# samuelkriegerbonini-dev/AstroBurst

Measured on AMD Instinct MI355X. Metric: MPix/s sigma-clipped stack+stretch, 64x4096x4096 f32, higher is better.
Workload: dtype f32

## Files before the change

### astroburst_amd/csrc/affine.hip

```cpp
#include "ab_common.hpp"

#include <algorithm>
#include <condition_variable>
#include <mutex>
#include <thread>
#include <array>
#include <atomic>
#include <chrono>
#include <cmath>
#include <thread>

int ab_phase_correlate_device(ab_ctx *ctx, const float *ref, int64_t ref_rows, int64_t ref_cols, int64_t ref_ld, const float *tgt,
                              int64_t tgt_rows, int64_t tgt_cols, int64_t tgt_ld, double *dx, double *dy, double *confidence);

namespace {

constexpr size_t kMaxStars = 120;
constexpr double kTriangleTolerance = 0.02;
constexpr size_t kMinMatchesAffine = 6, kMinMatchesRigid = 4;
constexpr size_t kRansacIterations = 2000;
constexpr double kRansacInlierPx = 3.0, kDetectionSigma = 3.5, kMinTriangleSide = 15.0;
constexpr uint32_t kMinVotes = 1;
constexpr double kMinInlierRatio = 0.20, kMaxResidualPx = 5.0, kMaxOffsetFraction = 0.40, kMaxRotationDeg = 30.0;
constexpr double kMinScale = 0.70, kMaxScale = 1.40;
// ... 373 lines not shown
    __syncthreads();
    if (ok) {
        unsigned int base = block_base;
        for (int w = 0; w < wv; ++w) base += wave_cnt[w];
        out[base + (unsigned int)__builtin_popcountll(m & ((1ull << lane) - 1ull))] = tri;
        if (bin_hist) atomicAdd(&lhist[tri.bin], 1u);
    }
    if (bin_hist) {
        __syncthreads();
        for (int b = threadIdx.x; b < kTriBins; b += kTriBlock)
            if (lhist[b]) atomicAdd(&bin_hist[b], lhist[b]);
    }
}

constexpr int kScanThreads = 256, kScanPer = kTriBins / kScanThreads;
__device__ __forceinline__ void tri_bin_scan_body(unsigned int *__restrict__ hist, unsigned int *__restrict__ off ,
                                                            unsigned int *__restrict__ cursor) {
    __shared__ unsigned int wave_tot[kScanThreads / 64];
    const int t = threadIdx.x, lane = t & 63, wv = t >> 6;
    unsigned int h[kScanPer], s = 0;
#pragma unroll
    for (int j = 0; j < kScanPer; j += 4) {
        const uint4 q = *reinterpret_cast<const uint4 *>(hist + kScanPer * t + j);
        h[j] = q.x, h[j + 1] = q.y, h[j + 2] = q.z, h[j + 3] = q.w;
        s += q.x + q.y + q.z + q.w;
    }
    unsigned int inc = s;
#pragma unroll
    for (int o = 1; o < 64; o <<= 1) {
        const unsigned int u = __shfl_up(inc, o, 64);
        if (lane >= o) inc += u;
    }
    if (lane == 63) wave_tot[wv] = inc;
    __syncthreads();
    unsigned int base = 0;
    for (int i = 0; i < wv; ++i) base += wave_tot[i];
    unsigned int e = base + inc - s;
#pragma unroll
    for (int j = 0; j < kScanPer; ++j) {
        off[kScanPer * t + j] = e;
        cursor[kScanPer * t + j] = e;
        hist[kScanPer * t + j] = 0;
        e += h[j];
    }
    if (t == kScanThreads - 1) off[kTriBins] = e;
}

__device__ __forceinline__ void tri_scatter_body(const DTri *__restrict__ in, const unsigned int *__restrict__ n_p, unsigned int *cursor,
                                                           DTri *__restrict__ sorted) {
    __shared__ unsigned int cnt[kTriBins];
    const unsigned int n = *n_p, i = blockIdx.x * kTriBlock + threadIdx.x;
    if (blockIdx.x * kTriBlock >= n) return;
    for (int b = threadIdx.x; b < kTriBins; b += kTriBlock) cnt[b] = 0;
    __syncthreads();
    DTri t = {0.0, 0.0, 0u, 0u};
    unsigned int rank = 0;
    if (i < n) {
// ... 165 lines not shown
    __syncthreads();
    unsigned int *mine = votes_out + (size_t)(blockIdx.x % (unsigned int)copies) * (kVoteDim * kVoteDim);
    for (int row = wv; row < kVoteDim; row += kVoteWaves) {
        const unsigned int v = votes[row * kVoteLdsStride + lane];
        if (v) atomicAdd(&mine[row * kVoteDim + lane], v);
    }
}

constexpr int kTriGroupMax = 8;
struct TriGroup {
    int n;
    int limit[kTriGroupMax];
    DTri *raw[kTriGroupMax], *sorted[kTriGroupMax];
    unsigned int *count[kTriGroupMax], *bin_hist[kTriGroupMax], *bin_off[kTriGroupMax], *cursor[kTriGroupMax], *votes[kTriGroupMax];
};
__global__ __launch_bounds__(kTriBlock) void tri_build_kernel(const StarXY stars, int limit, DTri *__restrict__ out, unsigned int *count,
                                                         unsigned int *__restrict__ bin_hist, unsigned int *__restrict__ votes_to_clear, int vote_words) { AB_LATENCY_KERNEL_PRIO();
    tri_build_body(stars.xy, limit, out, count, bin_hist, votes_to_clear, vote_words);
}
__global__ __launch_bounds__(kTriBlock) void tri_build_many_kernel(const TriGroup g, const StarXY *__restrict__ stars, int vote_words) { AB_LATENCY_KERNEL_PRIO();
    const int f = blockIdx.y;
    tri_build_body(stars[f].xy, g.limit[f], g.raw[f], g.count[f], g.bin_hist[f], g.votes[f], vote_words);
}
__global__ __launch_bounds__(kScanThreads) void tri_bin_scan_kernel(unsigned int *__restrict__ hist, unsigned int *__restrict__ off, unsigned int *__restrict__ cursor) { AB_LATENCY_KERNEL_PRIO();
    tri_bin_scan_body(hist, off, cursor);
}
__global__ __launch_bounds__(kScanThreads) void tri_bin_scan_many_kernel(const TriGroup g) { AB_LATENCY_KERNEL_PRIO();
    const int f = blockIdx.y;
    tri_bin_scan_body(g.bin_hist[f], g.bin_off[f], g.cursor[f]);
}
__global__ __launch_bounds__(kTriBlock) void tri_scatter_kernel(const DTri *__restrict__ in, const unsigned int *__restrict__ n_p, unsigned int *cursor,
                                                           DTri *__restrict__ sorted) { AB_LATENCY_KERNEL_PRIO();
    tri_scatter_body(in, n_p, cursor, sorted);
}
__global__ __launch_bounds__(kTriBlock) void tri_scatter_many_kernel(const TriGroup g) { AB_LATENCY_KERNEL_PRIO();
    const int f = blockIdx.y;
    tri_scatter_body(g.raw[f], g.count[f], g.cursor[f], g.sorted[f]);
}
__global__ __launch_bounds__(64) void tri_vote_kernel(const DTri *__restrict__ rt_sorted, const unsigned int *__restrict__ nr_p, const DTri *__restrict__ tt_sorted,
                                                      const unsigned int *__restrict__ bin_off, unsigned int *__restrict__ votes_out, int copies,
                                                      const RefGroup *__restrict__ groups, unsigned int *__restrict__ tgt_count_to_clear) { AB_LATENCY_KERNEL_PRIO();
    tri_vote_body(rt_sorted, nr_p, tt_sorted, bin_off, votes_out, copies, groups, tgt_count_to_clear);
}
__global__ __launch_bounds__(64) void tri_vote_many_kernel(const TriGroup g, const DTri *__restrict__ rt_sorted, const unsigned int *__restrict__ nr_p, int copies,
                                                           const RefGroup *__restrict__ groups) { AB_LATENCY_KERNEL_PRIO();
    const int f = blockIdx.y;
    tri_vote_body(rt_sorted, nr_p, g.sorted[f], g.bin_off[f], g.votes[f], copies, groups, g.count[f]);
}
__global__ __launch_bounds__(kVoteWaves * 64) void tri_vote_wide_kernel(const DTri *__restrict__ rt_sorted, const unsigned int *__restrict__ nr_p, const DTri *__restrict__ tt_sorted,
                                                                        const unsigned int *__restrict__ bin_off, unsigned int *__restrict__ votes_out, int copies,
                                                                        const RefGroup *__restrict__ groups, unsigned int *__restrict__ tgt_count_to_clear, unsigned int slices) { AB_LATENCY_KERNEL_PRIO();
    tri_vote_wide_body(rt_sorted, nr_p, tt_sorted, bin_off, votes_out, copies, groups, tgt_count_to_clear, slices);
}
__global__ __launch_bounds__(kVoteWaves * 64) void tri_vote_wide_many_kernel(const TriGroup g, const DTri *__restrict__ rt_sorted, const unsigned int *__restrict__ nr_p, int copies,
                                                                             const RefGroup *__restrict__ groups, unsigned int slices) { AB_LATENCY_KERNEL_PRIO();
    const int f = blockIdx.y;
    tri_vote_wide_body(rt_sorted, nr_p, g.sorted[f], g.bin_off[f], g.votes[f], copies, groups, g.count[f], slices);
}
unsigned int vote_wide_slices() {
    static const unsigned int v = [] {
        const char *e = ab_dev_env("AB_VOTE_SLICES");
        const int x = e ? atoi(e) : 8;
        return (unsigned int)(x < 1 ? 1 : (x > 8 ? 8 : x));
    }();
    return v;
}
bool vote_wide() {
    static const bool on = [] {
        const char *e = ab_dev_env("AB_VOTE_WAVES");
        return !(e && atoi(e) == 1);
    }();
    return on;
}

__global__ __launch_bounds__(256) void votes_reduce_many_kernel(const TriGroup g, int copies, uint32_t *__restrict__ out) { AB_LATENCY_KERNEL_PRIO();
    const int f = blockIdx.y, i = blockIdx.x * 256 + threadIdx.x;
    if (i >= kVoteDim * kVoteDim) return;
    uint32_t s = 0;
    for (int c = 0; c < copies; ++c) s += g.votes[f][(size_t)c * kVoteDim * kVoteDim + i];
    out[(size_t)f * kVoteDim * kVoteDim + i] = s;
}

struct MatchWs {
    DTri *ref_tris, *ref_sorted, *tgt_tris, *tgt_sorted;
    unsigned int *counts;
    unsigned int *bin_hist, *bin_off, *cursor;
    unsigned int *votes;
    RefGroup *groups;
};

int match_ws(ab_ctx *ctx, MatchWs *w) {
    const size_t tri_bytes = (size_t)kMaxTris * sizeof(DTri), vote_bytes = (size_t)kVoteCopiesMax * kVoteDim * kVoteDim * sizeof(unsigned int);
    const size_t bin_words = 64 + 3 * (size_t)kTriBins + 64;
    const size_t group_bytes = (size_t)((kMaxTris + 63) / 64) * sizeof(RefGroup);
    const size_t total = 4 * tri_bytes + bin_words * sizeof(unsigned int) + vote_bytes + group_bytes;
// ... 110 lines not shown
    int max_limit = 0;
    for (int f = 0; f < G; ++f) {
        const int limit = (int)std::min<size_t>(stars[f].size(), kTriLimit);
        w.g.limit[f] = limit;
        max_limit = std::max(max_limit, limit);
        for (int i = 0; i < limit; ++i) {
            hs[f].xy[2 * i] = stars[f][i][0];
            hs[f].xy[2 * i + 1] = stars[f][i][1];
        }
    }
    for (int f = 0; f < G; ++f) votes[f].assign((size_t)kVoteDim * kVoteDim, 0u);
    if (max_limit < 3) return AB_OK;
    AB_HIP(ctx, hipMemcpyAsync(w.stars, hs, stars_bytes, hipMemcpyHostToDevice, ctx->stream));
    const int total = max_limit * max_limit * max_limit, blocks = std::max((total + kTriBlock - 1) / kTriBlock, (vote_words + kTriBlock - 1) / kTriBlock);
    hipLaunchKernelGGL(tri_build_many_kernel, dim3(blocks, G), dim3(kTriBlock), 0, ctx->stream, w.g, (const StarXY *)w.stars, vote_words);
    hipLaunchKernelGGL(tri_bin_scan_many_kernel, dim3(1, G), dim3(kScanThreads), 0, ctx->stream, w.g);
    hipLaunchKernelGGL(tri_scatter_many_kernel, dim3((kMaxTris + kTriBlock - 1) / kTriBlock, G), dim3(kTriBlock), 0, ctx->stream, w.g);
    if (vote_wide())
        hipLaunchKernelGGL(tri_vote_wide_many_kernel, dim3((kVoteItemsMax + kVoteWaves - 1) / kVoteWaves, G), dim3(kVoteWaves * 64), 0, ctx->stream, w.g,
                           (const DTri *)ref_ws.ref_sorted, (const unsigned int *)ref_ws.counts, copies, (const RefGroup *)ref_ws.groups, vote_wide_slices());
    else
        hipLaunchKernelGGL(tri_vote_many_kernel, dim3(kVoteBlocks, G), dim3(64), 0, ctx->stream, w.g, (const DTri *)ref_ws.ref_sorted, (const unsigned int *)ref_ws.counts,
                           copies, (const RefGroup *)ref_ws.groups);
    uint32_t *hv = (uint32_t *)((char *)pin + stars_bytes);
    hipLaunchKernelGGL(votes_reduce_many_kernel, dim3((kVoteDim * kVoteDim + 255) / 256, G), dim3(256), 0, ctx->stream, w.g, copies, hv);
    AB_HIP(ctx, hipGetLastError());
    AB_HIP(ctx, hipStreamSynchronize(ctx->stream));
    for (int f = 0; f < G; ++f) votes[f].assign(hv + (size_t)f * per_frame_words, hv + (size_t)(f + 1) * per_frame_words);
    return AB_OK;
}

int frame_stars(ab_ctx *ctx, const float *img, int64_t rows, int64_t cols, std::vector<Pt> *out, const ab_pixel_xf *xf = nullptr,
                const double *bg = nullptr, const ab_frame_cand *cand = nullptr ) {
    std::vector<ab_detected_star> stars;
    double m, s;
    if (xf && bg) {
        const double b2[1][2] = {{bg[0], bg[1]}};
        AB_TRY(ab_detect_stars_group_device(ctx, &img, 1, rows, cols, kDetectionSigma, xf, b2, kMaxStars, &stars, cand));
    } else {
        AB_TRY(ab_detect_stars_device(ctx, img, rows, cols, cols, kDetectionSigma, &stars, &m, &s, xf ? *xf : ab_pixel_xf(), kMaxStars,
// ... 447 lines not shown
```

### astroburst_amd/csrc/detect.hip

```cpp
#include "ab_common.hpp"
#include "block_select.hpp"
#include "tile_bucket.hpp"
#include "tile_stream.hpp"

#include <algorithm>
#include <cfloat>
#include <cmath>
#include <chrono>
#include <condition_variable>
#include <thread>

namespace {

constexpr double kMadToSigma = 1.4826;

struct FrameDev {
    ab_pixel_xf xf;
    double bg_median, bg_sigma, threshold;
    unsigned int finite;
    unsigned int pad;
};

constexpr int kCandCap = 2048;
struct TileCand {
// ... 1356 lines not shown
    unsigned int *mask[kGroupMax], *counters[kGroupMax];
    CompStat *st[kGroupMax];
    CompRec *rec[kGroupMax];
    unsigned int ncomp[kGroupMax];
    unsigned int comp_cap;
    int chained;
    int *blist[kGroupMax];
    unsigned int *lcnt[kGroupMax];
    size_t plist_stride, blist_stride;
    int tiled;
    int mask_pitch;
    int recs;
    size_t rec_stride;
    unsigned int *sel[kGroupMax];
    unsigned int *selout[kGroupMax];
    const uint2 *cand_ent[kGroupMax];
    const unsigned int *cand_cnt[kGroupMax];
    const float *cand_cut[kGroupMax];
    int tile_h, tile_w;
};

static inline bool selection_cut_too_close(const std::vector<ab_detected_star> &stars, size_t max_keep, unsigned int selected, unsigned int candidates,
                                           unsigned int cut_key) {
    if (candidates <= selected || cut_key == 0 || stars.empty() || stars.size() < max_keep) return false;
    unsigned long long bits;
    const double fl = stars.back().flux;
    memcpy(&bits, &fl, sizeof bits);
    const unsigned long long key = (bits >> 32) + 1ull;
    return key < (unsigned long long)cut_key + 2ull;
}

constexpr unsigned int kSelKeep = 480, kSelCap = 544;
__device__ __forceinline__ unsigned int sel_key(const CompStat &c) {
    const bool ok = c.npix >= 3 && c.npix <= 5000 && c.first_interior != 0x7fffffff && c.flux > 0.0;
    return ok ? (unsigned int)((unsigned long long)__double_as_longlong(c.flux) >> 32) + 1u : 0u;
}
constexpr int kSelThreads = 256, kSelSub = 2048;
__device__ __forceinline__ unsigned int sel_digit(unsigned int k) {
    constexpr int kBase = (1023 - 64) << 20;
    const int d = ((int)k - kBase) >> 16;
    return (unsigned int)(d < 0 ? 0 : (d > 2047 ? 2047 : d));
}
__device__ __forceinline__ void sel_find_digit(const unsigned int *hist, int nb, unsigned int want, int tid, unsigned int *digit, unsigned int *above) {
    unsigned int run = 0, found = 0, ab = 0;
    bool done = false;
    for (int base = nb - 64; base >= 0 && !done; base -= 64) {
        const unsigned int c = hist[base + 63 - tid];
        unsigned int incl = c;
#pragma unroll
        for (int off = 1; off < 64; off <<= 1) {
            const unsigned int o = __shfl_up(incl, off, 64);
            if (tid >= off) incl += o;
        }
        const unsigned long long hit = __ballot(run + incl >= want);
        if (hit) {
            const int l = __builtin_ctzll(hit);
            ab = run + __shfl(incl, l, 64) - __shfl(c, l, 64);
            found = (unsigned int)(base + 63 - l);
            done = true;
        } else {
            run += __shfl(incl, 63, 64);
        }
    }
    *digit = found;
    *above = ab;
}
__global__ __launch_bounds__(kSelThreads) void comp_select_many_kernel(const DetGroup g) { AB_LATENCY_KERNEL_PRIO();
    const int f = blockIdx.x, tid = threadIdx.x;
    unsigned int n = g.ncomp[f];
    if (g.chained && !g.recs) {
        n = g.counters[f][0];
        if (tid == 0) g.selout[f][2] = n;
        if (n > g.comp_cap) n = 0;
    }
    const CompStat *__restrict__ st = g.st[f];
    unsigned int *__restrict__ sel = g.sel[f];
    __shared__ unsigned int hist[2048];
    __shared__ unsigned int sub_key[kSelSub], sub_idx[kSelSub];
    __shared__ unsigned int s_ncand, s_d0, s_above, s_count, s_nsub, s_prefix, s_want, s_ge, s_take;
    __shared__ unsigned int seg_n[kRecRegions], seg_t0[kRecRegions + 1];
    const int nseg = g.recs ? kRecRegions : 1;
    const unsigned int seg_stride = g.recs ? (unsigned int)g.rec_stride : 0u;
    for (unsigned int b = tid; b < 2048; b += kSelThreads) hist[b] = 0;
    if (tid == 0) s_ncand = s_d0 = s_above = s_count = s_nsub = s_prefix = s_want = s_ge = s_take = 0;
    if (g.recs) {
        const unsigned int flagw = g.counters[f][3];
        const bool overflow = (flagw & 1u) != 0;
        if (tid == 0 && g.chained) g.selout[f][4] = flagw >> 1;
        if (tid < kRecRegions) {
            const unsigned int cnt = g.lcnt[f][(2 * kRegions + tid) * kRegionPitch];
            seg_n[tid] = overflow ? 0u : (cnt < seg_stride ? cnt : seg_stride);
        }
        __syncthreads();
        if (tid == 0) {
            unsigned int t = 0, total = 0;
            for (int sg = 0; sg < kRecRegions; ++sg) {
                seg_t0[sg] = t;
                t += (seg_n[sg] + kSelThreads - 1) / kSelThreads;
                total += seg_n[sg];
            }
            seg_t0[kRecRegions] = t;
            g.selout[f][2] = overflow ? g.comp_cap + 1u : total;
        }
    } else if (tid == 0) {
        seg_n[0] = n;
        seg_t0[0] = 0;
        seg_t0[1] = (n + kSelThreads - 1) / kSelThreads;
    }
    __syncthreads();
    const unsigned int trips = seg_t0[nseg];
    constexpr unsigned int kSelIlp = 8;
    auto scan = [&](auto &&consume) {
        if (g.recs) {
            unsigned int most = 0;
#pragma unroll
            for (int sg = 0; sg < kRecRegions; ++sg) most = max(most, seg_n[sg]);
            for (unsigned int j = tid; j < most; j += kSelThreads) {
                unsigned int k[kRecRegions];
#pragma unroll
                for (int sg = 0; sg < kRecRegions; ++sg) k[sg] = j < seg_n[sg] ? sel_key(st[(unsigned int)sg * seg_stride + j]) : 0u;
#pragma unroll
                for (int sg = 0; sg < kRecRegions; ++sg) consume(k[sg], (unsigned int)sg * seg_stride + j);
            }
            return;
        }
        for (unsigned int t0 = 0; t0 < trips; t0 += kSelIlp) {
            unsigned int k[kSelIlp];
#pragma unroll
            for (unsigned int u = 0; u < kSelIlp; ++u) {
                const unsigned int i = (t0 + u) * kSelThreads + tid;
                k[u] = i < n ? sel_key(st[i]) : 0u;
            }
#pragma unroll
            for (unsigned int u = 0; u < kSelIlp; ++u) consume(k[u], (t0 + u) * kSelThreads + tid);
        }
    };
    unsigned int mine = 0;
    scan([&](unsigned int k, unsigned int) {
        mine += k ? 1u : 0u;
        if (k) atomicAdd(&hist[sel_digit(k)], 1u);
    });
#pragma unroll
    for (int off = 32; off >= 1; off >>= 1) mine += __shfl_xor(mine, off, 64);
    if ((tid & 63) == 0 && mine) atomicAdd(&s_ncand, mine);
    __syncthreads();
    const unsigned int ncand = s_ncand;
    const bool all = ncand <= kSelKeep;
    if (!all && tid < 64) {
        unsigned int d0, above;
        sel_find_digit(hist, 2048, kSelKeep, tid, &d0, &above);
        if (tid == 0) {
            s_d0 = d0;
            s_above = above;
            s_take = above + hist[d0] <= kSelCap ? 1u : 0u;
        }
    }
    __syncthreads();
    const unsigned int d0 = s_d0, above = s_above;
    const bool take_bin = s_take != 0;
    scan([&](unsigned int k, unsigned int i) {
        if (!k) return;
        const unsigned int dg = sel_digit(k);
        if (all || dg > d0 || (take_bin && dg == d0)) {
            const unsigned int at = atomicAdd(&s_count, 1u);
            if (at < kSelCap) sel[at] = i;
        } else if (dg == d0) {
            const unsigned int at = atomicAdd(&s_nsub, 1u);
            if (at < (unsigned int)kSelSub) {
                sub_key[at] = k;
                sub_idx[at] = i;
            }
        }
    });
    __syncthreads();
    const unsigned int nsub = s_nsub;
    constexpr unsigned int kDigitBase = (unsigned int)((1023 - 64) << 20);
    unsigned int cut_key = all ? 0u : (take_bin ? (d0 ? kDigitBase + (d0 << 16) : 1u) : kDigitBase + ((d0 + 1u) << 16));
    if (!all && !take_bin && nsub <= (unsigned int)kSelSub) {
        const unsigned int want0 = kSelKeep - above;
        const unsigned int strips = (nsub + kSelThreads - 1) / kSelThreads;
        unsigned int prefix = 0, mask = 0, want = want0;
        const int shifts[3] = {21, 10, 0}, bits[3] = {11, 11, 10};
        for (int lv = 0; lv < 3; ++lv) {
            const unsigned int nb = 1u << bits[lv];
            for (unsigned int b = tid; b < nb; b += kSelThreads) hist[b] = 0;
            __syncthreads();
            for (unsigned int t = 0; t < strips; ++t) {
                const unsigned int j = t * kSelThreads + tid;
                const unsigned int k = j < nsub ? sub_key[j] : 0u;
                if (j < nsub && (k & mask) == prefix) atomicAdd(&hist[(k >> shifts[lv]) & (nb - 1)], 1u);
            }
            __syncthreads();
            if (tid < 64) {
                unsigned int dg, ab;
                sel_find_digit(hist, (int)nb, want, tid, &dg, &ab);
                if (tid == 0) {
                    s_prefix = prefix | (dg << shifts[lv]);
                    s_want = want - ab;
                }
            }
            __syncthreads();
            prefix = s_prefix;
            want = s_want;
            mask |= (nb - 1) << shifts[lv];
        }
        unsigned int thr = prefix;
        unsigned int ge = 0;
        for (unsigned int j = tid; j < nsub; j += kSelThreads) ge += sub_key[j] >= thr ? 1u : 0u;
#pragma unroll
        for (int off = 32; off >= 1; off >>= 1) ge += __shfl_xor(ge, off, 64);
        if ((tid & 63) == 0 && ge) atomicAdd(&s_ge, ge);
        __syncthreads();
        if (above + s_ge > kSelCap) thr += 1;
        cut_key = thr;
        for (unsigned int j = tid; j < nsub; j += kSelThreads) {
            if (sub_key[j] >= thr) {
                const unsigned int at = atomicAdd(&s_count, 1u);
                if (at < kSelCap) sel[at] = sub_idx[j];
            }
        }
    }
    __syncthreads();
    if (tid == 0) {
        const unsigned int m = min(s_count, kSelCap);
        g.counters[f][2] = m;
        g.selout[f][0] = m;
        g.selout[f][3] = cut_key;
        g.selout[f][1] = s_count > kSelCap ? 0xffffffffu : ncand;
    }
}

__global__ __launch_bounds__(kInitBlock) void label_init_kernel(const float *__restrict__ img, int rows, int cols, int64_t ld, double threshold_arg,
                                                                const ab_pixel_xf xf_arg, int *__restrict__ parent, unsigned int *__restrict__ mask,
// ... 998 lines not shown
    unsigned int *mask = nullptr;
    const int mask_pitch = (int)((cols + 31) / 32 * 32);
    const size_t mask_words = (size_t)rows * (size_t)(mask_pitch / 32) + 2, roots_words = (size_t)root_cap + 4;
    AB_TRY(ab_workspace(ctx, AB_WS_DETECT_PARENT, (size_t)G * P * sizeof(int), (void **)&parent));
    AB_TRY(ab_workspace(ctx, AB_WS_DETECT_CID, (size_t)G * P * sizeof(int), (void **)&cid));
    AB_TRY(ab_workspace(ctx, AB_WS_DETECT_ROOTS, (size_t)G * roots_words * sizeof(int), (void **)&roots));
    const bool tiled = !ctx->label_legacy;
    const bool bg_tiles = tiled && cand && cand[0].ent && !ctx->label_pixelwise && !ctx->detect_no_recs && !ctx->detect_full_records && !ctx->detect_midjoin &&
                          4 * max_keep <= (size_t)kSelKeep;
    const int tile_h = bg_tiles ? kBgRows : kTileH, tile_w = bg_tiles ? kBgT : kTileW, tile_slots = bg_tiles ? kBgSlots : kTileSlots;
    const int64_t tiles_x = (cols + tile_w - 1) / tile_w, tiles_y = bg_tiles ? ((rows + kBgT - 1) / kBgT) * kBgSub : (rows + tile_h - 1) / tile_h, ntile = tiles_x * tiles_y;
    const size_t tiles_per_region = ((size_t)ntile + kRegions - 1) / kRegions;
    const size_t plist_stride = bg_tiles ? 0 : tiles_per_region * (size_t)(kTileH * kTileW), blist_stride = tiles_per_region * (size_t)(tile_w + 2 * tile_h);
    const size_t plist_ints = tiled ? (size_t)kRegions * plist_stride : (size_t)P, blist_ints = tiled ? (size_t)kRegions * blist_stride : 0;
    const size_t lcnt_words = tiled ? (size_t)(2 * kRegions + kRecRegions) * kRegionPitch : 0;
    AB_TRY(ab_workspace(ctx, AB_WS_DETECT_LIST, (size_t)G * (plist_ints + blist_ints + lcnt_words) * sizeof(int), (void **)&plist));
    AB_TRY(ab_workspace(ctx, AB_WS_DETECT_MASK, (size_t)G * mask_words * sizeof(unsigned int), (void **)&mask));
    DetGroup g;
    memset(&g, 0, sizeof g);
    g.n = G;
    bool vec_ok = (P & 3) == 0;
    unsigned int *counters = (unsigned int *)(roots + (size_t)G * root_cap);
    for (int f = 0; f < G; ++f) {
        g.img[f] = imgs[f];
        g.bg_median[f] = bg[f][0];
        g.threshold[f] = bg[f][0] + sigma_threshold * bg[f][1];
        g.xf[f] = xf[f];
        g.parent[f] = parent + (size_t)f * P;
        g.cid[f] = cid + (size_t)f * P;
        g.plist[f] = plist + (size_t)f * plist_ints;
        g.blist[f] = plist + (size_t)G * plist_ints + (size_t)f * blist_ints;
        g.lcnt[f] = (unsigned int *)(plist + (size_t)G * (plist_ints + blist_ints)) + (size_t)f * lcnt_words;
        g.roots[f] = roots + (size_t)f * root_cap;
        g.mask[f] = mask + (size_t)f * mask_words;
        g.counters[f] = counters + 4 * f;
        vec_ok = vec_ok && ((uintptr_t)imgs[f] & 15) == 0;
    }
    const int cus = ctx->cu_count > 0 ? ctx->cu_count : 256;
    const int gl = tiled ? std::max(kRegions, (cus * 2 / kRegions) * kRegions) : cus * 2;
    const bool select = !ctx->detect_full_records && 4 * max_keep <= (size_t)kSelKeep;
    const bool chained = select && !ctx->detect_midjoin;
    const size_t rec_stride = (((size_t)ntile + kRecRegions - 1) / kRecRegions) * (size_t)tile_slots, rec_cap = (size_t)kRecRegions * rec_stride;
    const bool recs = chained && tiled && !ctx->label_pixelwise && !ctx->detect_no_recs && rec_cap <= (size_t)root_cap;
    AB_CHECK(ctx, !bg_tiles || recs, "detect_stars: the background-tile labelling needs the records form (%zu records for %u roots)", rec_cap, root_cap);
    const unsigned int comp_cap = recs ? (unsigned int)rec_cap : (unsigned int)std::min<int64_t>(root_cap, (int64_t)1 << 18);
    void *pin = nullptr;
    unsigned int *selout = nullptr;
    if (chained) {
        void *cbuf = nullptr;
        AB_TRY(ab_workspace(ctx, AB_WS_DETECT_COMPS, (size_t)G * comp_cap * sizeof(CompStat) + (size_t)G * kSelCap * sizeof(unsigned int), &cbuf));
        CompStat *dstat = (CompStat *)cbuf;
        unsigned int *dsel = (unsigned int *)(dstat + (size_t)G * comp_cap);
        AB_TRY(ab_pinned(ctx, (size_t)G * kSelCap * sizeof(CompRec) + (size_t)G * 8 * sizeof(unsigned int), &pin));
        selout = (unsigned int *)((CompRec *)pin + (size_t)G * kSelCap);
        for (int f = 0; f < G; ++f) {
            g.rec[f] = (CompRec *)pin + (size_t)f * kSelCap;
            g.st[f] = dstat + (size_t)f * comp_cap;
            g.sel[f] = dsel + (size_t)f * kSelCap;
            g.selout[f] = selout + 8 * f;
            for (int k = 0; k < 8; ++k) selout[8 * f + k] = 0;
        }
        g.comp_cap = comp_cap;
        g.chained = 1;
    }
    AB_HIP(ctx, hipMemsetAsync(counters, 0, (size_t)G * 4 * sizeof(unsigned int), ctx->stream));
    g.tiled = tiled ? 1 : 0;
    g.tile_h = tile_h;
    g.tile_w = tile_w;
    for (int f = 0; f < G; ++f) {
        const bool has = bg_tiles && cand[f].ent;
        g.cand_ent[f] = has ? (const uint2 *)cand[f].ent : nullptr;
        g.cand_cnt[f] = has ? cand[f].cnt : nullptr;
        g.cand_cut[f] = has ? cand[f].cut : nullptr;
    }
    g.mask_pitch = mask_pitch;
    g.recs = recs ? 1 : 0;
    g.rec_stride = rec_stride;
    g.plist_stride = plist_stride;
    g.blist_stride = blist_stride;
    if (tiled) AB_HIP(ctx, hipMemsetAsync(g.lcnt[0], 0, (size_t)G * lcnt_words * sizeof(unsigned int), ctx->stream));
    if (tiled) {
        if (bg_tiles)
            hipLaunchKernelGGL(label_bgtile_many_kernel, dim3((unsigned)ntile, (unsigned)G), dim3(kBgThreads), 0, ctx->stream, g, (int)rows, (int)cols);
        else if (recs)
            hipLaunchKernelGGL((label_tile_many_kernel<true, true>), dim3((unsigned)ntile, (unsigned)G), dim3(kTileThreads), 0, ctx->stream, g, (int)rows, (int)cols);
        else if (ctx->label_pixelwise)
            hipLaunchKernelGGL((label_tile_many_kernel<false, false>), dim3((unsigned)ntile, (unsigned)G), dim3(kTileThreads), 0, ctx->stream, g, (int)rows, (int)cols);
        else
            hipLaunchKernelGGL((label_tile_many_kernel<true, false>), dim3((unsigned)ntile, (unsigned)G), dim3(kTileThreads), 0, ctx->stream, g, (int)rows, (int)cols);
        hipLaunchKernelGGL(label_border_many_kernel, dim3(gl, G), dim3(256), 0, ctx->stream, g, (int)rows, (int)cols);
    } else {
        hipLaunchKernelGGL(label_init_many_kernel, dim3((unsigned)((P + kInitSub * kInitRounds - 1) / (kInitSub * kInitRounds)), (unsigned)G), dim3(kInitBlock), 0, ctx->stream, g,
                           (int)rows, (int)cols, cols, (int)vec_ok);
        hipLaunchKernelGGL(label_merge_many_kernel, dim3(gl, G), dim3(256), 0, ctx->stream, g, (int)rows, (int)cols);
    }
    if (recs) {
        hipLaunchKernelGGL(comp_merge_many_kernel, dim3(4 * kRecRegions, G), dim3(256), 0, ctx->stream, g);
    } else {
        hipLaunchKernelGGL(roots_many_kernel, dim3(gl, G), dim3(kRootsBlock), 0, ctx->stream, g, chained ? comp_cap : root_cap);
    }
    AB_HIP(ctx, hipGetLastError());
    if (chained) {
        if (!recs) hipLaunchKernelGGL(comp_stats_many_kernel, dim3(gl, G), dim3(256), 0, ctx->stream, g, (int)rows, (int)cols, cols);
        hipLaunchKernelGGL(comp_select_many_kernel, dim3(G), dim3(kSelThreads), 0, ctx->stream, g);
        hipLaunchKernelGGL(comp_moments_many_kernel, dim3((kSelCap + 4 * kMomPerWave - 1) / (4 * kMomPerWave), G), dim3(256), 0, ctx->stream, g, (int)cols, cols);
        AB_HIP(ctx, hipGetLastError());
        AB_HIP(ctx, hipStreamSynchronize(ctx->stream));
        bool redo[kGroupMax] = {};
        unsigned int sel_m[kGroupMax] = {}, sel_ncand[kGroupMax] = {}, sel_ncomp[kGroupMax] = {};
        size_t sel_stars[kGroupMax] = {};
        for (int f = 0; f < G; ++f) {
            const unsigned int m = selout[8 * f], ncand = selout[8 * f + 1], ncomp = selout[8 * f + 2], cut_key = selout[8 * f + 3];
            if (bg_tiles) ab_count_fallback(ctx, AB_FB_LABEL_TILES_DENSE, selout[8 * f + 4]);
            sel_m[f] = m;
            sel_ncand[f] = ncand;
            sel_ncomp[f] = ncomp;
            AB_CHECK(ctx, m <= kSelCap, "detect_stars: the selection of frame %d holds %u components", f, m);
            AB_CHECK(ctx, ncomp <= root_cap, "detect_stars: %u components exceed the table capacity", ncomp);
            if (ncomp > comp_cap) {
// ... 25 lines not shown
    AB_TRY(ab_pinned(ctx, (size_t)G * 4 * sizeof(unsigned int), &pin));
    AB_HIP(ctx, hipMemcpyAsync(pin, counters, (size_t)G * 4 * sizeof(unsigned int), hipMemcpyDeviceToHost, ctx->stream));
    AB_HIP(ctx, hipStreamSynchronize(ctx->stream));
    size_t total = 0, off[kGroupMax + 1];
    unsigned int max_nc = 0;
    for (int f = 0; f < G; ++f) {
        g.ncomp[f] = ((const unsigned int *)pin)[4 * f];
        AB_CHECK(ctx, g.ncomp[f] <= root_cap, "detect_stars: %u components exceed the table capacity", g.ncomp[f]);
        off[f] = total;
        total += g.ncomp[f];
        max_nc = std::max(max_nc, g.ncomp[f]);
    }
    off[G] = total;
    if (total == 0) return AB_OK;
    void *cbuf = nullptr;
    AB_TRY(ab_workspace(ctx, AB_WS_DETECT_COMPS, total * sizeof(CompStat) + (size_t)G * kSelCap * sizeof(unsigned int), &cbuf));
    CompStat *dstat = (CompStat *)cbuf;
    unsigned int *dsel = (unsigned int *)(dstat + total);
    const size_t rec_count = select ? (size_t)G * kSelCap : total;
    AB_TRY(ab_pinned(ctx, rec_count * sizeof(CompRec) + (size_t)G * 4 * sizeof(unsigned int), &pin));
    selout = (unsigned int *)((CompRec *)pin + rec_count);
    for (int f = 0; f < G; ++f) {
        g.rec[f] = (CompRec *)pin + (select ? (size_t)f * kSelCap : off[f]);
        g.st[f] = dstat + off[f];
        g.sel[f] = select ? dsel + (size_t)f * kSelCap : nullptr;
        g.selout[f] = selout + 4 * f;
        selout[4 * f] = selout[4 * f + 1] = selout[4 * f + 3] = 0;
    }
    hipLaunchKernelGGL(comp_init_many_kernel, dim3((max_nc + 255) / 256, G), dim3(256), 0, ctx->stream, g);
    hipLaunchKernelGGL(comp_stats_many_kernel, dim3(gl, G), dim3(256), 0, ctx->stream, g, (int)rows, (int)cols, cols);
#ifdef AB_DEV_ABLATION
    if (ab_dev_env("AB_ABLATE_MOMENTS")) {
        const int v = atoi(ab_dev_env("AB_ABLATE_MOMENTS"));
        AB_HIP(ctx, hipMemcpyToSymbol(HIP_SYMBOL(g_mom_ablate), &v, sizeof v));
    }
#endif
    if (select) {
        hipLaunchKernelGGL(comp_select_many_kernel, dim3(G), dim3(kSelThreads), 0, ctx->stream, g);
        hipLaunchKernelGGL(comp_moments_many_kernel, dim3((kSelCap + 4 * kMomPerWave - 1) / (4 * kMomPerWave), G), dim3(256), 0, ctx->stream, g, (int)cols, cols);
    } else {
        hipLaunchKernelGGL(comp_moments_many_kernel, dim3((max_nc + 4 * kMomPerWave - 1) / (4 * kMomPerWave), G), dim3(256), 0, ctx->stream, g, (int)cols, cols);
    }
    AB_HIP(ctx, hipGetLastError());
    AB_HIP(ctx, hipStreamSynchronize(ctx->stream));
    bool redo[kGroupMax] = {};
    for (int f = 0; f < G; ++f) {
        if (!select) {
            finish_stars((const CompRec *)pin + off[f], g.ncomp[f], bg[f][1], max_keep, &stars[f]);
            continue;
        }
        const unsigned int m = selout[4 * f], ncand = selout[4 * f + 1], cut_key = selout[4 * f + 3];
        AB_CHECK(ctx, m <= kSelCap, "detect_stars: the selection of frame %d holds %u components", f, m);
        finish_stars(g.rec[f], m, bg[f][1], max_keep, &stars[f]);
// ... 157 lines not shown
```

Before: 111,700.

## Fuse triangle scan and vote reduce into last-arriver tails; parallelize component selection

```diff
diff --git a/astroburst_amd/csrc/affine.hip b/astroburst_amd/csrc/affine.hip
--- a/astroburst_amd/csrc/affine.hip
+++ b/astroburst_amd/csrc/affine.hip
@@ -411,16 +411,25 @@
 }
 
 constexpr int kScanThreads = 256, kScanPer = kTriBins / kScanThreads;
-__device__ __forceinline__ void tri_bin_scan_body(unsigned int *__restrict__ hist, unsigned int *__restrict__ off ,
+template <bool IN_LAUNCH>
+__device__ __forceinline__ void tri_bin_scan_body(unsigned int *hist, unsigned int *__restrict__ off ,
                                                             unsigned int *__restrict__ cursor) {
     __shared__ unsigned int wave_tot[kScanThreads / 64];
     const int t = threadIdx.x, lane = t & 63, wv = t >> 6;
     unsigned int h[kScanPer], s = 0;
+    if constexpr (IN_LAUNCH) {
 #pragma unroll
-    for (int j = 0; j < kScanPer; j += 4) {
-        const uint4 q = *reinterpret_cast<const uint4 *>(hist + kScanPer * t + j);
-        h[j] = q.x, h[j + 1] = q.y, h[j + 2] = q.z, h[j + 3] = q.w;
-        s += q.x + q.y + q.z + q.w;
+        for (int j = 0; j < kScanPer; ++j) {
+            h[j] = __hip_atomic_load(hist + kScanPer * t + j, __ATOMIC_RELAXED, __HIP_MEMORY_SCOPE_AGENT);
+            s += h[j];
+        }
+    } else {
+#pragma unroll
+        for (int j = 0; j < kScanPer; j += 4) {
+            const uint4 q = *reinterpret_cast<const uint4 *>(hist + kScanPer * t + j);
+            h[j] = q.x, h[j + 1] = q.y, h[j + 2] = q.z, h[j + 3] = q.w;
+            s += q.x + q.y + q.z + q.w;
+        }
     }
     unsigned int inc = s;
 #pragma unroll
@@ -437,7 +446,8 @@
     for (int j = 0; j < kScanPer; ++j) {
         off[kScanPer * t + j] = e;
         cursor[kScanPer * t + j] = e;
-        hist[kScanPer * t + j] = 0;
+        if constexpr (IN_LAUNCH) __hip_atomic_store(hist + kScanPer * t + j, 0u, __ATOMIC_RELAXED, __HIP_MEMORY_SCOPE_AGENT);
+        else hist[kScanPer * t + j] = 0;
         e += h[j];
     }
     if (t == kScanThreads - 1) off[kTriBins] = e;
@@ -633,6 +643,30 @@
     DTri *raw[kTriGroupMax], *sorted[kTriGroupMax];
     unsigned int *count[kTriGroupMax], *bin_hist[kTriGroupMax], *bin_off[kTriGroupMax], *cursor[kTriGroupMax], *votes[kTriGroupMax];
 };
+__device__ __forceinline__ bool tri_last_arriver(unsigned int *ticket, unsigned int expected) {
+    __shared__ unsigned int s_last;
+    asm volatile("s_waitcnt vmcnt(0)" ::: "memory");
+    __syncthreads();
+    if (threadIdx.x == 0) {
+        __builtin_amdgcn_fence(__ATOMIC_RELEASE, "agent");
+        asm volatile("s_waitcnt vmcnt(0)" ::: "memory");
+        const unsigned int t = __hip_atomic_fetch_add(ticket, 1u, __ATOMIC_RELAXED, __HIP_MEMORY_SCOPE_AGENT);
+        s_last = t + 1u == expected ? 1u : 0u;
+        if (t + 1u == expected) __hip_atomic_store(ticket, 0u, __ATOMIC_RELAXED, __HIP_MEMORY_SCOPE_AGENT);
+    }
+    __syncthreads();
+    const bool last = s_last != 0;
+    if (last) __builtin_amdgcn_fence(__ATOMIC_ACQUIRE, "agent");
+    return last;
+}
+constexpr int kTicketBuild = 16, kTicketVote = 32;
+__device__ __forceinline__ void votes_reduce_tail(unsigned int *votes, int copies, uint32_t *__restrict__ out) {
+    for (int i = threadIdx.x; i < kVoteDim * kVoteDim; i += blockDim.x) {
+        uint32_t s = 0;
+        for (int c = 0; c < copies; ++c) s += __hip_atomic_load(votes + (size_t)c * kVoteDim * kVoteDim + i, __ATOMIC_RELAXED, __HIP_MEMORY_SCOPE_AGENT);
+        out[i] = s;
+    }
+}
 __global__ __launch_bounds__(kTriBlock) void tri_build_kernel(const StarXY stars, int limit, DTri *__restrict__ out, unsigned int *count,
                                                          unsigned int *__restrict__ bin_hist, unsigned int *__restrict__ votes_to_clear, int vote_words) { AB_LATENCY_KERNEL_PRIO();
     tri_build_body(stars.xy, limit, out, count, bin_hist, votes_to_clear, vote_words);
@@ -640,13 +674,11 @@
 __global__ __launch_bounds__(kTriBlock) void tri_build_many_kernel(const TriGroup g, const StarXY *__restrict__ stars, int vote_words) { AB_LATENCY_KERNEL_PRIO();
     const int f = blockIdx.y;
     tri_build_body(stars[f].xy, g.limit[f], g.raw[f], g.count[f], g.bin_hist[f], g.votes[f], vote_words);
+    static_assert(kScanThreads == kTriBlock, "the scan is a tail of the builder's workgroup");
+    if (tri_last_arriver(g.count[f] + kTicketBuild, gridDim.x)) tri_bin_scan_body<true>(g.bin_hist[f], g.bin_off[f], g.cursor[f]);
 }
 __global__ __launch_bounds__(kScanThreads) void tri_bin_scan_kernel(unsigned int *__restrict__ hist, unsigned int *__restrict__ off, unsigned int *__restrict__ cursor) { AB_LATENCY_KERNEL_PRIO();
-    tri_bin_scan_body(hist, off, cursor);
-}
-__global__ __launch_bounds__(kScanThreads) void tri_bin_scan_many_kernel(const TriGroup g) { AB_LATENCY_KERNEL_PRIO();
-    const int f = blockIdx.y;
-    tri_bin_scan_body(g.bin_hist[f], g.bin_off[f], g.cursor[f]);
+    tri_bin_scan_body<false>(hist, off, cursor);
 }
 __global__ __launch_bounds__(kTriBlock) void tri_scatter_kernel(const DTri *__restrict__ in, const unsigned int *__restrict__ n_p, unsigned int *cursor,
                                                            DTri *__restrict__ sorted) { AB_LATENCY_KERNEL_PRIO();
@@ -662,9 +694,10 @@
     tri_vote_body(rt_sorted, nr_p, tt_sorted, bin_off, votes_out, copies, groups, tgt_count_to_clear);
 }
 __global__ __launch_bounds__(64) void tri_vote_many_kernel(const TriGroup g, const DTri *__restrict__ rt_sorted, const unsigned int *__restrict__ nr_p, int copies,
-                                                           const RefGroup *__restrict__ groups) { AB_LATENCY_KERNEL_PRIO();
+                                                           const RefGroup *__restrict__ groups, uint32_t *__restrict__ out ) { AB_LATENCY_KERNEL_PRIO();
     const int f = blockIdx.y;
     tri_vote_body(rt_sorted, nr_p, g.sorted[f], g.bin_off[f], g.votes[f], copies, groups, g.count[f]);
+    if (tri_last_arriver(g.count[f] + kTicketVote, gridDim.x)) votes_reduce_tail(g.votes[f], copies, out + (size_t)f * kVoteDim * kVoteDim);
 }
 __global__ __launch_bounds__(kVoteWaves * 64) void tri_vote_wide_kernel(const DTri *__restrict__ rt_sorted, const unsigned int *__restrict__ nr_p, const DTri *__restrict__ tt_sorted,
                                                                         const unsigned int *__restrict__ bin_off, unsigned int *__restrict__ votes_out, int copies,
@@ -672,9 +705,11 @@
     tri_vote_wide_body(rt_sorted, nr_p, tt_sorted, bin_off, votes_out, copies, groups, tgt_count_to_clear, slices);
 }
 __global__ __launch_bounds__(kVoteWaves * 64) void tri_vote_wide_many_kernel(const TriGroup g, const DTri *__restrict__ rt_sorted, const unsigned int *__restrict__ nr_p, int copies,
-                                                                             const RefGroup *__restrict__ groups, unsigned int slices) { AB_LATENCY_KERNEL_PRIO();
+                                                                             const RefGroup *__restrict__ groups, unsigned int slices,
+                                                                             uint32_t *__restrict__ out ) { AB_LATENCY_KERNEL_PRIO();
     const int f = blockIdx.y;
     tri_vote_wide_body(rt_sorted, nr_p, g.sorted[f], g.bin_off[f], g.votes[f], copies, groups, g.count[f], slices);
+    if (tri_last_arriver(g.count[f] + kTicketVote, gridDim.x)) votes_reduce_tail(g.votes[f], copies, out + (size_t)f * kVoteDim * kVoteDim);
 }
 unsigned int vote_wide_slices() {
     static const unsigned int v = [] {
@@ -690,14 +725,6 @@
         return !(e && atoi(e) == 1);
     }();
     return on;
-}
-
-__global__ __launch_bounds__(256) void votes_reduce_many_kernel(const TriGroup g, int copies, uint32_t *__restrict__ out) { AB_LATENCY_KERNEL_PRIO();
-    const int f = blockIdx.y, i = blockIdx.x * 256 + threadIdx.x;
-    if (i >= kVoteDim * kVoteDim) return;
-    uint32_t s = 0;
-    for (int c = 0; c < copies; ++c) s += g.votes[f][(size_t)c * kVoteDim * kVoteDim + i];
-    out[(size_t)f * kVoteDim * kVoteDim + i] = s;
 }
 
 struct MatchWs {
@@ -838,16 +865,14 @@
     AB_HIP(ctx, hipMemcpyAsync(w.stars, hs, stars_bytes, hipMemcpyHostToDevice, ctx->stream));
     const int total = max_limit * max_limit * max_limit, blocks = std::max((total + kTriBlock - 1) / kTriBlock, (vote_words + kTriBlock - 1) / kTriBlock);
     hipLaunchKernelGGL(tri_build_many_kernel, dim3(blocks, G), dim3(kTriBlock), 0, ctx->stream, w.g, (const StarXY *)w.stars, vote_words);
-    hipLaunchKernelGGL(tri_bin_scan_many_kernel, dim3(1, G), dim3(kScanThreads), 0, ctx->stream, w.g);
     hipLaunchKernelGGL(tri_scatter_many_kernel, dim3((kMaxTris + kTriBlock - 1) / kTriBlock, G), dim3(kTriBlock), 0, ctx->stream, w.g);
+    uint32_t *hv = (uint32_t *)((char *)pin + stars_bytes);
     if (vote_wide())
         hipLaunchKernelGGL(tri_vote_wide_many_kernel, dim3((kVoteItemsMax + kVoteWaves - 1) / kVoteWaves, G), dim3(kVoteWaves * 64), 0, ctx->stream, w.g,
-                           (const DTri *)ref_ws.ref_sorted, (const unsigned int *)ref_ws.counts, copies, (const RefGroup *)ref_ws.groups, vote_wide_slices());
+                           (const DTri *)ref_ws.ref_sorted, (const unsigned int *)ref_ws.counts, copies, (const RefGroup *)ref_ws.groups, vote_wide_slices(), hv);
     else
         hipLaunchKernelGGL(tri_vote_many_kernel, dim3(kVoteBlocks, G), dim3(64), 0, ctx->stream, w.g, (const DTri *)ref_ws.ref_sorted, (const unsigned int *)ref_ws.counts,
-                           copies, (const RefGroup *)ref_ws.groups);
-    uint32_t *hv = (uint32_t *)((char *)pin + stars_bytes);
-    hipLaunchKernelGGL(votes_reduce_many_kernel, dim3((kVoteDim * kVoteDim + 255) / 256, G), dim3(256), 0, ctx->stream, w.g, copies, hv);
+                           copies, (const RefGroup *)ref_ws.groups, hv);
     AB_HIP(ctx, hipGetLastError());
     AB_HIP(ctx, hipStreamSynchronize(ctx->stream));
     for (int f = 0; f < G; ++f) votes[f].assign(hv + (size_t)f * per_frame_words, hv + (size_t)(f + 1) * per_frame_words);
diff --git a/astroburst_amd/csrc/detect.hip b/astroburst_amd/csrc/detect.hip
--- a/astroburst_amd/csrc/detect.hip
+++ b/astroburst_amd/csrc/detect.hip
@@ -1394,6 +1394,8 @@
     size_t rec_stride;
     unsigned int *sel[kGroupMax];
     unsigned int *selout[kGroupMax];
+    unsigned int *selstate[kGroupMax];
+    unsigned int *selsub[kGroupMax];
     const uint2 *cand_ent[kGroupMax];
     const unsigned int *cand_cnt[kGroupMax];
     const float *cand_cut[kGroupMax];
@@ -1415,7 +1417,8 @@
     const bool ok = c.npix >= 3 && c.npix <= 5000 && c.first_interior != 0x7fffffff && c.flux > 0.0;
     return ok ? (unsigned int)((unsigned long long)__double_as_longlong(c.flux) >> 32) + 1u : 0u;
 }
-constexpr int kSelThreads = 256, kSelSub = 2048;
+constexpr int kSelThreads = 256, kSelSub = 2048, kSelWgs = 16, kSelBins = 2048;
+constexpr int kSelStateWords = kSelBins + 64;
 __device__ __forceinline__ unsigned int sel_digit(unsigned int k) {
     constexpr int kBase = (1023 - 64) << 20;
     const int d = ((int)k - kBase) >> 16;
@@ -1445,101 +1448,136 @@
     *digit = found;
     *above = ab;
 }
+__device__ __forceinline__ bool sel_last_arriver(unsigned int *ticket, unsigned int expected) {
+    __shared__ unsigned int s_last;
+    asm volatile("s_waitcnt vmcnt(0)" ::: "memory");
+    __syncthreads();
+    if (threadIdx.x == 0) {
+        __builtin_amdgcn_fence(__ATOMIC_RELEASE, "agent");
+        asm volatile("s_waitcnt vmcnt(0)" ::: "memory");
+        s_last = __hip_atomic_fetch_add(ticket, 1u, __ATOMIC_RELAXED, __HIP_MEMORY_SCOPE_AGENT) + 1u == expected ? 1u : 0u;
+    }
+    __syncthreads();
+    const bool last = s_last != 0;
+    if (last) __builtin_amdgcn_fence(__ATOMIC_ACQUIRE, "agent");
+    return last;
+}
 __global__ __launch_bounds__(kSelThreads) void comp_select_many_kernel(const DetGroup g) { AB_LATENCY_KERNEL_PRIO();
-    const int f = blockIdx.x, tid = threadIdx.x;
+    const int f = blockIdx.y, tid = threadIdx.x;
     unsigned int n = g.ncomp[f];
     if (g.chained && !g.recs) {
         n = g.counters[f][0];
-        if (tid == 0) g.selout[f][2] = n;
         if (n > g.comp_cap) n = 0;
     }
     const CompStat *__restrict__ st = g.st[f];
     unsigned int *__restrict__ sel = g.sel[f];
-    __shared__ unsigned int hist[2048];
-    __shared__ unsigned int sub_key[kSelSub], sub_idx[kSelSub];
-    __shared__ unsigned int s_ncand, s_d0, s_above, s_count, s_nsub, s_prefix, s_want, s_ge, s_take;
-    __shared__ unsigned int seg_n[kRecRegions], seg_t0[kRecRegions + 1];
-    const int nseg = g.recs ? kRecRegions : 1;
+    unsigned int *ghist = g.selstate[f], *gncand = ghist + kSelBins, *ticket = ghist + kSelBins + 32;
+    __shared__ unsigned int hist[256];
+    __shared__ unsigned int wave_tot[kSelThreads / 64];
+    __shared__ unsigned int s_d0, s_above, s_count, s_nsub, s_prefix, s_want, s_ge, s_take;
+    __shared__ unsigned int seg_n[kRecRegions];
+    const unsigned int nseg = g.recs ? kRecRegions : 1;
     const unsigned int seg_stride = g.recs ? (unsigned int)g.rec_stride : 0u;
-    for (unsigned int b = tid; b < 2048; b += kSelThreads) hist[b] = 0;
-    if (tid == 0) s_ncand = s_d0 = s_above = s_count = s_nsub = s_prefix = s_want = s_ge = s_take = 0;
+    if (tid == 0) s_d0 = s_above = s_count = s_nsub = s_prefix = s_want = s_ge = s_take = 0;
+    if (tid < kRecRegions) seg_n[tid] = 0;
+    __syncthreads();
+    bool overflow = false;
+    unsigned int flagw = 0;
     if (g.recs) {
-        const unsigned int flagw = g.counters[f][3];
-        const bool overflow = (flagw & 1u) != 0;
-        if (tid == 0 && g.chained) g.selout[f][4] = flagw >> 1;
+        flagw = g.counters[f][3];
+        overflow = (flagw & 1u) != 0;
         if (tid < kRecRegions) {
             const unsigned int cnt = g.lcnt[f][(2 * kRegions + tid) * kRegionPitch];
             seg_n[tid] = overflow ? 0u : (cnt < seg_stride ? cnt : seg_stride);
         }
-        __syncthreads();
-        if (tid == 0) {
-            unsigned int t = 0, total = 0;
-            for (int sg = 0; sg < kRecRegions; ++sg) {
-                seg_t0[sg] = t;
-                t += (seg_n[sg] + kSelThreads - 1) / kSelThreads;
-                total += seg_n[sg];
-            }
-            seg_t0[kRecRegions] = t;
-            g.selout[f][2] = overflow ? g.comp_cap + 1u : total;
-        }
     } else if (tid == 0) {
         seg_n[0] = n;
-        seg_t0[0] = 0;
-        seg_t0[1] = (n + kSelThreads - 1) / kSelThreads;
     }
     __syncthreads();
-    const unsigned int trips = seg_t0[nseg];
+    unsigned int most = 0, total = 0;
+#pragma unroll
+    for (int sg = 0; sg < kRecRegions; ++sg) {
+        most = max(most, seg_n[sg]);
+        total += seg_n[sg];
+    }
+    const unsigned int items = nseg * most;
     constexpr unsigned int kSelIlp = 8;
-    auto scan = [&](auto &&consume) {
-        if (g.recs) {
-            unsigned int most = 0;
-#pragma unroll
-            for (int sg = 0; sg < kRecRegions; ++sg) most = max(most, seg_n[sg]);
-            for (unsigned int j = tid; j < most; j += kSelThreads) {
-                unsigned int k[kRecRegions];
-#pragma unroll
-                for (int sg = 0; sg < kRecRegions; ++sg) k[sg] = j < seg_n[sg] ? sel_key(st[(unsigned int)sg * seg_stride + j]) : 0u;
-#pragma unroll
-                for (int sg = 0; sg < kRecRegions; ++sg) consume(k[sg], (unsigned int)sg * seg_stride + j);
+    auto scan = [&](unsigned int first, unsigned int step, auto &&consume) {
+        for (unsigned int it0 = first; it0 < items; it0 += kSelIlp * step) {
+            unsigned int k[kSelIlp], idx[kSelIlp];
+#pragma unroll
+            for (unsigned int u = 0; u < kSelIlp; ++u) {
+                const unsigned int it = it0 + u * step;
+                k[u] = 0u;
+                idx[u] = 0u;
+                if (it < items) {
+                    const unsigned int sg = it / most, j = it - sg * most;
+                    idx[u] = sg * seg_stride + j;
+                    if (j < seg_n[sg]) k[u] = sel_key(st[idx[u]]);
+                }
             }
-            return;
-        }
-        for (unsigned int t0 = 0; t0 < trips; t0 += kSelIlp) {
-            unsigned int k[kSelIlp];
-#pragma unroll
-            for (unsigned int u = 0; u < kSelIlp; ++u) {
-                const unsigned int i = (t0 + u) * kSelThreads + tid;
-                k[u] = i < n ? sel_key(st[i]) : 0u;
-            }
-#pragma unroll
-            for (unsigned int u = 0; u < kSelIlp; ++u) consume(k[u], (t0 + u) * kSelThreads + tid);
+#pragma unroll
+            for (unsigned int u = 0; u < kSelIlp; ++u)
+                if (k[u]) consume(k[u], idx[u]);
         }
     };
     unsigned int mine = 0;
-    scan([&](unsigned int k, unsigned int) {
-        mine += k ? 1u : 0u;
-        if (k) atomicAdd(&hist[sel_digit(k)], 1u);
+    scan(blockIdx.x * kSelThreads + tid, gridDim.x * kSelThreads, [&](unsigned int k, unsigned int) {
+        ++mine;
+        __hip_atomic_fetch_add(&ghist[sel_digit(k)], 1u, __ATOMIC_RELAXED, __HIP_MEMORY_SCOPE_AGENT);
     });
 #pragma unroll
     for (int off = 32; off >= 1; off >>= 1) mine += __shfl_xor(mine, off, 64);
-    if ((tid & 63) == 0 && mine) atomicAdd(&s_ncand, mine);
-    __syncthreads();
-    const unsigned int ncand = s_ncand;
+    if ((tid & 63) == 0 && mine) __hip_atomic_fetch_add(gncand, mine, __ATOMIC_RELAXED, __HIP_MEMORY_SCOPE_AGENT);
+    if (!sel_last_arriver(ticket, gridDim.x)) return;
+    if (tid == 0 && g.chained) {
+        if (g.recs) {
+            g.selout[f][4] = flagw >> 1;
+            g.selout[f][2] = overflow ? g.comp_cap + 1u : total;
+        } else {
+            g.selout[f][2] = g.counters[f][0];
+        }
+    }
+    const unsigned int ncand = __hip_atomic_load(gncand, __ATOMIC_RELAXED, __HIP_MEMORY_SCOPE_AGENT);
     const bool all = ncand <= kSelKeep;
-    if (!all && tid < 64) {
-        unsigned int d0, above;
-        sel_find_digit(hist, 2048, kSelKeep, tid, &d0, &above);
-        if (tid == 0) {
-            s_d0 = d0;
-            s_above = above;
-            s_take = above + hist[d0] <= kSelCap ? 1u : 0u;
+    {
+        constexpr int kPer = kSelBins / kSelThreads;
+        unsigned int h[kPer], sum = 0;
+#pragma unroll
+        for (int j = 0; j < kPer; ++j) {
+            h[j] = __hip_atomic_load(ghist + (kSelBins - 1 - (kPer * tid + j)), __ATOMIC_RELAXED, __HIP_MEMORY_SCOPE_AGENT);
+            sum += h[j];
+        }
+        unsigned int inc = sum;
+        const int lane = tid & 63, wv = tid >> 6;
+#pragma unroll
+        for (int o = 1; o < 64; o <<= 1) {
+            const unsigned int u = __shfl_up(inc, o, 64);
+            if (lane >= o) inc += u;
+        }
+        if (lane == 63) wave_tot[wv] = inc;
+        __syncthreads();
+        unsigned int run = inc - sum;
+        for (int i = 0; i < wv; ++i) run += wave_tot[i];
+        if (!all && run < kSelKeep && run + sum >= kSelKeep) {
+            bool found = false;
+#pragma unroll
+            for (int j = 0; j < kPer; ++j) {
+                if (!found && run + h[j] >= kSelKeep) {
+                    found = true;
+                    s_d0 = (unsigned int)(kSelBins - 1 - (kPer * tid + j));
+                    s_above = run;
+                    s_take = run + h[j] <= kSelCap ? 1u : 0u;
+                }
+                if (!found) run += h[j];
+            }
         }
     }
     __syncthreads();
     const unsigned int d0 = s_d0, above = s_above;
     const bool take_bin = s_take != 0;
-    scan([&](unsigned int k, unsigned int i) {
-        if (!k) return;
+    unsigned int *sub_key = g.selsub[f], *sub_idx = sub_key + kSelSub;
+    scan(tid, kSelThreads, [&](unsigned int k, unsigned int i) {
         const unsigned int dg = sel_digit(k);
         if (all || dg > d0 || (take_bin && dg == d0)) {
             const unsigned int at = atomicAdd(&s_count, 1u);
@@ -1558,45 +1596,49 @@
     unsigned int cut_key = all ? 0u : (take_bin ? (d0 ? kDigitBase + (d0 << 16) : 1u) : kDigitBase + ((d0 + 1u) << 16));
     if (!all && !take_bin && nsub <= (unsigned int)kSelSub) {
         const unsigned int want0 = kSelKeep - above;
-        const unsigned int strips = (nsub + kSelThreads - 1) / kSelThreads;
+        constexpr int kSubPer = kSelSub / kSelThreads;
+        unsigned int key[kSubPer];
+#pragma unroll
+        for (int t = 0; t < kSubPer; ++t) {
+            const unsigned int j = (unsigned int)t * kSelThreads + tid;
+            key[t] = j < nsub ? sub_key[j] : 0u;
+        }
         unsigned int prefix = 0, mask = 0, want = want0;
-        const int shifts[3] = {21, 10, 0}, bits[3] = {11, 11, 10};
-        for (int lv = 0; lv < 3; ++lv) {
-            const unsigned int nb = 1u << bits[lv];
-            for (unsigned int b = tid; b < nb; b += kSelThreads) hist[b] = 0;
+        for (int shift = 24; shift >= 0; shift -= 8) {
+            hist[tid] = 0;
             __syncthreads();
-            for (unsigned int t = 0; t < strips; ++t) {
-                const unsigned int j = t * kSelThreads + tid;
-                const unsigned int k = j < nsub ? sub_key[j] : 0u;
-                if (j < nsub && (k & mask) == prefix) atomicAdd(&hist[(k >> shifts[lv]) & (nb - 1)], 1u);
-            }
+#pragma unroll
+            for (int t = 0; t < kSubPer; ++t)
+                if (key[t] && (key[t] & mask) == prefix) atomicAdd(&hist[(key[t] >> shift) & 255u], 1u);
             __syncthreads();
             if (tid < 64) {
                 unsigned int dg, ab;
-                sel_find_digit(hist, (int)nb, want, tid, &dg, &ab);
+                sel_find_digit(hist, 256, want, tid, &dg, &ab);
                 if (tid == 0) {
-                    s_prefix = prefix | (dg << shifts[lv]);
+                    s_prefix = prefix | (dg << shift);
                     s_want = want - ab;
                 }
             }
             __syncthreads();
             prefix = s_prefix;
             want = s_want;
-            mask |= (nb - 1) << shifts[lv];
+            mask |= 255u << shift;
         }
         unsigned int thr = prefix;
         unsigned int ge = 0;
-        for (unsigned int j = tid; j < nsub; j += kSelThreads) ge += sub_key[j] >= thr ? 1u : 0u;
+#pragma unroll
+        for (int t = 0; t < kSubPer; ++t) ge += key[t] >= thr ? 1u : 0u;
 #pragma unroll
         for (int off = 32; off >= 1; off >>= 1) ge += __shfl_xor(ge, off, 64);
         if ((tid & 63) == 0 && ge) atomicAdd(&s_ge, ge);
         __syncthreads();
         if (above + s_ge > kSelCap) thr += 1;
         cut_key = thr;
-        for (unsigned int j = tid; j < nsub; j += kSelThreads) {
-            if (sub_key[j] >= thr) {
+#pragma unroll
+        for (int t = 0; t < kSubPer; ++t) {
+            if (key[t] >= thr) {
                 const unsigned int at = atomicAdd(&s_count, 1u);
-                if (at < kSelCap) sel[at] = sub_idx[j];
+                if (at < kSelCap) sel[at] = sub_idx[(unsigned int)t * kSelThreads + tid];
             }
         }
     }
@@ -2625,13 +2667,16 @@
     const size_t plist_stride = bg_tiles ? 0 : tiles_per_region * (size_t)(kTileH * kTileW), blist_stride = tiles_per_region * (size_t)(tile_w + 2 * tile_h);
     const size_t plist_ints = tiled ? (size_t)kRegions * plist_stride : (size_t)P, blist_ints = tiled ? (size_t)kRegions * blist_stride : 0;
     const size_t lcnt_words = tiled ? (size_t)(2 * kRegions + kRecRegions) * kRegionPitch : 0;
-    AB_TRY(ab_workspace(ctx, AB_WS_DETECT_LIST, (size_t)G * (plist_ints + blist_ints + lcnt_words) * sizeof(int), (void **)&plist));
+    const size_t zero_words = ((size_t)G * (lcnt_words + 4 + kSelStateWords) + 63) / 64 * 64;
+    unsigned int *zero_block = nullptr;
+    AB_TRY(ab_workspace(ctx, AB_WS_DETECT_LIST, (zero_words + (size_t)G * (plist_ints + blist_ints)) * sizeof(int), (void **)&zero_block));
+    plist = (int *)(zero_block + zero_words);
     AB_TRY(ab_workspace(ctx, AB_WS_DETECT_MASK, (size_t)G * mask_words * sizeof(unsigned int), (void **)&mask));
     DetGroup g;
     memset(&g, 0, sizeof g);
     g.n = G;
     bool vec_ok = (P & 3) == 0;
-    unsigned int *counters = (unsigned int *)(roots + (size_t)G * root_cap);
+    unsigned int *counters = zero_block + (size_t)G * lcnt_words;
     for (int f = 0; f < G; ++f) {
         g.img[f] = imgs[f];
         g.bg_median[f] = bg[f][0];
@@ -2641,10 +2686,11 @@
         g.cid[f] = cid + (size_t)f * P;
         g.plist[f] = plist + (size_t)f * plist_ints;
         g.blist[f] = plist + (size_t)G * plist_ints + (size_t)f * blist_ints;
-        g.lcnt[f] = (unsigned int *)(plist + (size_t)G * (plist_ints + blist_ints)) + (size_t)f * lcnt_words;
+        g.lcnt[f] = zero_block + (size_t)f * lcnt_words;
         g.roots[f] = roots + (size_t)f * root_cap;
         g.mask[f] = mask + (size_t)f * mask_words;
         g.counters[f] = counters + 4 * f;
+        g.selstate[f] = counters + 4 * (size_t)G + (size_t)f * kSelStateWords;
         vec_ok = vec_ok && ((uintptr_t)imgs[f] & 15) == 0;
     }
     const int cus = ctx->cu_count > 0 ? ctx->cu_count : 256;
@@ -2659,7 +2705,7 @@
     unsigned int *selout = nullptr;
     if (chained) {
         void *cbuf = nullptr;
-        AB_TRY(ab_workspace(ctx, AB_WS_DETECT_COMPS, (size_t)G * comp_cap * sizeof(CompStat) + (size_t)G * kSelCap * sizeof(unsigned int), &cbuf));
+        AB_TRY(ab_workspace(ctx, AB_WS_DETECT_COMPS, (size_t)G * comp_cap * sizeof(CompStat) + (size_t)G * (kSelCap + 2 * kSelSub) * sizeof(unsigned int), &cbuf));
         CompStat *dstat = (CompStat *)cbuf;
         unsigned int *dsel = (unsigned int *)(dstat + (size_t)G * comp_cap);
         AB_TRY(ab_pinned(ctx, (size_t)G * kSelCap * sizeof(CompRec) + (size_t)G * 8 * sizeof(unsigned int), &pin));
@@ -2668,13 +2714,14 @@
             g.rec[f] = (CompRec *)pin + (size_t)f * kSelCap;
             g.st[f] = dstat + (size_t)f * comp_cap;
             g.sel[f] = dsel + (size_t)f * kSelCap;
+            g.selsub[f] = dsel + (size_t)G * kSelCap + (size_t)f * 2 * kSelSub;
             g.selout[f] = selout + 8 * f;
             for (int k = 0; k < 8; ++k) selout[8 * f + k] = 0;
         }
         g.comp_cap = comp_cap;
         g.chained = 1;
     }
-    AB_HIP(ctx, hipMemsetAsync(counters, 0, (size_t)G * 4 * sizeof(unsigned int), ctx->stream));
+    AB_HIP(ctx, hipMemsetAsync(zero_block, 0, zero_words * sizeof(unsigned int), ctx->stream));
     g.tiled = tiled ? 1 : 0;
     g.tile_h = tile_h;
     g.tile_w = tile_w;
@@ -2689,7 +2736,6 @@
     g.rec_stride = rec_stride;
     g.plist_stride = plist_stride;
     g.blist_stride = blist_stride;
-    if (tiled) AB_HIP(ctx, hipMemsetAsync(g.lcnt[0], 0, (size_t)G * lcnt_words * sizeof(unsigned int), ctx->stream));
     if (tiled) {
         if (bg_tiles)
             hipLaunchKernelGGL(label_bgtile_many_kernel, dim3((unsigned)ntile, (unsigned)G), dim3(kBgThreads), 0, ctx->stream, g, (int)rows, (int)cols);
@@ -2713,7 +2759,7 @@
     AB_HIP(ctx, hipGetLastError());
     if (chained) {
         if (!recs) hipLaunchKernelGGL(comp_stats_many_kernel, dim3(gl, G), dim3(256), 0, ctx->stream, g, (int)rows, (int)cols, cols);
-        hipLaunchKernelGGL(comp_select_many_kernel, dim3(G), dim3(kSelThreads), 0, ctx->stream, g);
+        hipLaunchKernelGGL(comp_select_many_kernel, dim3(kSelWgs, G), dim3(kSelThreads), 0, ctx->stream, g);
         hipLaunchKernelGGL(comp_moments_many_kernel, dim3((kSelCap + 4 * kMomPerWave - 1) / (4 * kMomPerWave), G), dim3(256), 0, ctx->stream, g, (int)cols, cols);
         AB_HIP(ctx, hipGetLastError());
         AB_HIP(ctx, hipStreamSynchronize(ctx->stream));
@@ -2769,7 +2815,7 @@
     off[G] = total;
     if (total == 0) return AB_OK;
     void *cbuf = nullptr;
-    AB_TRY(ab_workspace(ctx, AB_WS_DETECT_COMPS, total * sizeof(CompStat) + (size_t)G * kSelCap * sizeof(unsigned int), &cbuf));
+    AB_TRY(ab_workspace(ctx, AB_WS_DETECT_COMPS, total * sizeof(CompStat) + (size_t)G * (kSelCap + 2 * kSelSub) * sizeof(unsigned int), &cbuf));
     CompStat *dstat = (CompStat *)cbuf;
     unsigned int *dsel = (unsigned int *)(dstat + total);
     const size_t rec_count = select ? (size_t)G * kSelCap : total;
@@ -2779,6 +2825,7 @@
         g.rec[f] = (CompRec *)pin + (select ? (size_t)f * kSelCap : off[f]);
         g.st[f] = dstat + off[f];
         g.sel[f] = select ? dsel + (size_t)f * kSelCap : nullptr;
+        g.selsub[f] = dsel + (size_t)G * kSelCap + (size_t)f * 2 * kSelSub;
         g.selout[f] = selout + 4 * f;
         selout[4 * f] = selout[4 * f + 1] = selout[4 * f + 3] = 0;
     }
@@ -2791,7 +2838,7 @@
     }
 #endif
     if (select) {
-        hipLaunchKernelGGL(comp_select_many_kernel, dim3(G), dim3(kSelThreads), 0, ctx->stream, g);
+        hipLaunchKernelGGL(comp_select_many_kernel, dim3(kSelWgs, G), dim3(kSelThreads), 0, ctx->stream, g);
         hipLaunchKernelGGL(comp_moments_many_kernel, dim3((kSelCap + 4 * kMomPerWave - 1) / (4 * kMomPerWave), G), dim3(256), 0, ctx->stream, g, (int)cols, cols);
     } else {
         hipLaunchKernelGGL(comp_moments_many_kernel, dim3((max_nc + 4 * kMomPerWave - 1) / (4 * kMomPerWave), G), dim3(256), 0, ctx->stream, g, (int)cols, cols);
```

After: 88970. 20.4% lower.
